# yeyupiaoling/PPASR

Hardware: AMD Instinct MI355X
Metric: audio-seconds/s (RTF^-1) Conformer-streaming fbank, batch32 per GPU, ctc_greedy (higher is better)
Workload: dtype f32; 1 GPU; configs[1]: Conformer streaming (configs/conformer.yml), fbank-80, 32 x 10 s utterances per GPU, V=4233, ctc_greedy, features resident in HBM -> token ids + scores on device; global_batch=32, frames=1000, decoder=ctc_greedy, parallelism=utterance-dp1, pipelined=False, gemm=f32

## Files before the change

### ppasr_amd/csrc/front_fused.hip

```cpp
#include <utility>

#include "conformer_kernels.h"
#include "launch.h"

namespace ppasr {

namespace {
constexpr int kGroupRow[5] = {2, 0, 1, 4, 3};
constexpr int kTapCol[5] = {2, 0, 1, 4, 3};
constexpr int kFactor[5] = {2, 0, 1, 3, 1};
constexpr int quad_slab(int t) { return 4 * kFactor[t / 5] + kFactor[t % 5]; }
constexpr int quad_target(int t) {
  const int g = t / 5, k = t % 5;
  if (g == 0) return k == 0 ? 4 : k <= 2 ? 5 : 4;
  const int a = (g == 1 || g == 2) ? 0 : 2;
  return k == 0 ? (a == 0 ? 5 : 4) : k <= 2 ? a : a + 1;
}
constexpr int quad_fold_src(int t) {
  return t == 1 || t == 5 || t == 21 || t == 23 ? 4 : t == 3 || t == 11 || t == 13 ? 5 : -1;
}
constexpr int quad_fold_mask(int t) {
  return t == 1 ? 0xf : t == 3 ? 0x5 : t == 5 ? 0xa : t == 11 ? 0x2 : t == 13 ? 0x1 : t == 21 ? 0x8 : t == 23 ? 0x4 : 0;
}
constexpr bool quad_fold_clear(int t) { return t == 1 || t == 3 || t == 5 || t == 13 || t == 23; }
static_assert(quad_target(0) == 4 && quad_target(2) == 5 && quad_target(10) == 5 && quad_target(12) == 0 &&
                  quad_target(14) == 1 && quad_target(20) == 4 && quad_target(22) == 2 && quad_target(24) == 3,
              "chunk targets");

template <typename Fn, int... I>
__device__ __forceinline__ void static_for(std::integer_sequence<int, I...>, Fn&& fn) {
  (fn(std::integral_constant<int, I>{}), ...);
}

__host__ __device__ inline int quad_xs_stride(int F, int Q) { return F > 8 * Q + 3 ? F : 8 * Q + 3; }
}

template <bool FROM_Y1>
__device__ __forceinline__ void conv2_quad_body(const float* __restrict__ src, const FrontW& fw, float* __restrict__ out,
                                                int T, int F, int Tp, int F2, int M, int m0, const PadSkip& ps,
                                                const int* __restrict__ tile_tab) {
  constexpr int BP = 32, KC = 128, LD = KC + 4, G = KC / 8, NL = 2, N_CHUNKS = 25;
  constexpr int SLOT = BP * LD;
  const int P = (Tp + 1) >> 1;
  const int Q = (F2 + 1) >> 1;
  int r0 = m0 + blockIdx.x * BP, Mlim = M;
  if (tile_tab) {
    const int t = blockIdx.x, nb = tile_tab[0];
    const int* pre = tile_tab + 1;
    if (t >= pre[nb]) return;
    int lo = 0, hi = nb;
    while (hi - lo > 1) {
      const int mid = (lo + hi) >> 1;
      if (pre[mid] <= t) lo = mid;
      else hi = mid;
    }
    const int S = ps.Tp * ps.unit;
    r0 = lo * S + (t - pre[lo]) * BP;
    Mlim = min(M, (lo + 1) * S);
  } else if (pad_block_skippable(ps, r0, BP, M)) {
    return;
  }
  extern __shared__ __attribute__((aligned(16))) float smem[];
  float* const slot0 = smem;
  float* const slot1 = smem + SLOT;
  f32x4* const y2s = reinterpret_cast<f32x4*>(smem + 2 * SLOT);
  float* const w1s = smem + 2 * SLOT + 5 * NL * 4 * kThreads;
  float* const xs = w1s + 10 * 256;
  const int tid = threadIdx.x, lane = lane_id(), wave = wave_id();
  constexpr int tile_stride = 2 * 16 * G * 64;
  const f32x4* wbase = fw.conv2_wp + (size_t)wave * tile_stride;
  auto seg = [&](int h, int slab) { return wbase + (size_t)(16 * h + slab) * G * 64; };
  BRing<1> ring;
  ring_prime(ring, seg(0, quad_slab(0)), 0);
  const int c4 = tid & 31, rbase = tid >> 5;
  const int bp0 = r0 / Q;
  const int FX = quad_xs_stride(F, Q);
  uint32_t pb = 0;
  int yrow[FROM_Y1 ? NL : 1], yp4[FROM_Y1 ? NL : 1], yq4[FROM_Y1 ? NL : 1];
  if constexpr (!FROM_Y1) {
    for (int idx = tid; idx < 10 * 256; idx += kThreads) w1s[idx] = idx < 9 * 256 ? fw.conv1_w[idx] : fw.conv1_b[idx - 9 * 256];
    const int nbp = (min(r0 + BP, Mlim) - 1) / Q - bp0 + 1;
    for (int idx = tid; idx < nbp * 11 * FX; idx += kThreads) {
      const int fr_row = idx / FX, f = idx - fr_row * FX;
      const int bpl = fr_row / 11, fr = fr_row - 11 * bpl;
      const int bp = bp0 + bpl, b = bp / P, p = bp - b * P;
      const int t = min(8 * p + fr, T - 1);
      xs[idx] = f < F ? (src[((size_t)b * T + t) * F + f] - fw.cmvn_mean[f]) * fw.cmvn_istd[f] : 0.f;
    }
#pragma unroll
    for (int i = 0; i < NL; ++i) {
      const int m = r0 + rbase + 16 * i;
      const int bp = m / Q, q = m - bp * Q;
      const uint32_t v = m < Mlim ? (uint32_t)((bp - bp0) * 11 * FX + 8 * q) : 0xffffu;
      pb |= v << (16 * i);
    }
  } else {
#pragma unroll
    for (int i = 0; i < NL; ++i) {
      const int m = r0 + rbase + 16 * i;
      const int bp = m / Q, q = m - bp * Q, b = bp / P, p = bp - b * P;
      yrow[i] = b * T + 4 * p;
      yp4[i] = 4 * p;
      yq4[i] = m < Mlim ? 4 * q : -1;
    }
  }
  auto pbase = [&](int i) { return (int)((pb >> (16 * i)) & 0xffffu); };
  const int lds_off0 = rbase * LD + 4 * c4;
  float xv[9];
  f32x4 wv[3], bv, ya, yv;
  auto y1_step = [&](int i, int h, int r, int c, int step) {
    const int cc = h * 128 + 4 * c4;
    if constexpr (!FROM_Y1) {
      if (step == 0) {
        const int o = pbase(i);
        const float* p = xs + (o == 0xffff ? 0 : o) + 2 * r * FX + 2 * c;
#pragma unroll
        for (int ii = 0; ii < 3; ++ii)
#pragma unroll
          for (int jj = 0; jj < 3; ++jj) xv[ii * 3 + jj] = p[ii * FX + jj];
        ya = f32x4{0.f, 0.f, 0.f, 0.f};
      } else {
#pragma unroll
        for (int j = 3 * (step - 1); j < 3 * step; ++j)
#pragma unroll
          for (int e = 0; e < 4; ++e) ya[e] = fmaf(wv[j % 3][e], xv[j], ya[e]);
        if (step == 3) {
          ya += bv;
#pragma unroll
          for (int e = 0; e < 4; ++e) ya[e] = pbase(i) != 0xffff ? fmaxf(ya[e], 0.f) : 0.f;
        }
      }
      if (step < 3) {
#pragma unroll
        for (int j = 0; j < 3; ++j) wv[j] = *reinterpret_cast<const f32x4*>(w1s + (3 * step + j) * 256 + cc);
        if (step == 2) bv = *reinterpret_cast<const f32x4*>(w1s + 9 * 256 + cc);
      }
    } else {
      if (step == 0) {
        yv = f32x4{0.f, 0.f, 0.f, 0.f};
        if (yq4[i] >= 0 && yp4[i] + r < T && yq4[i] + c < F)
          yv = *reinterpret_cast<const f32x4*>(src + ((size_t)(yrow[i] + r) * F + yq4[i] + c) * 256 + cc);
      } else if (step == 3) {
        ya = yv;
      }
    }
  };
  auto put = [&](float* buf, int i, const f32x4& v) { *reinterpret_cast<f32x4*>(buf + lds_off0 + i * 16 * LD) = v; };
  auto y2row = [&](int c, int i) -> f32x4& { return y2s[(c * NL + i) * kThreads + tid]; };
  f32x4 z2[NL];
  auto build = [&](auto nc, int g, int h, float* buf) {
    constexpr int n = decltype(nc)::value, grp = n / 5, k = n % 5, r = kGroupRow[grp], c = kTapCol[k];
    const int i = g >> 2, step = g & 3;
    y1_step(i, h, r, c, step);
    if (step != 3) return;
    f32x4 v = ya;
    if constexpr (grp == 0) y2row(c, i) = ya;
    if constexpr (grp == 1 || grp == 3) v = ya - y2row(c, i);
    if constexpr (k == 0) {
      z2[i] = v;
      put(buf, i, v);
    } else if constexpr (k == 1 || k == 3) {
      put(buf, i, v - z2[i]);
    } else {
      put(buf, i, v);
    }
  };
  f32x16 acc[6][1][1];
#pragma unroll
  for (int a = 0; a < 6; ++a) acc_zero(acc[a]);
  auto fold = [&](auto tc, int g) {
    constexpr int t = decltype(tc)::value, fs = quad_fold_src(t), mask = quad_fold_mask(t);
    if constexpr (fs >= 0) {
      const int j = g - 4 * NL;
      int seen = 0;
#pragma unroll
      for (int o = 0; o < 4; ++o) {
        if (!((mask >> o) & 1)) continue;
        if (seen++ == j) {
#pragma unroll
          for (int e = 0; e < 16; ++e) asm volatile("v_add_f32 %0, %0, %1" : "+v"(acc[o][0][0][e]) : "v"(acc[fs][0][0][e]));
        }
      }
      if (quad_fold_clear(t) && j == 4) acc_zero(acc[fs]);
    }
  };
  __syncthreads();
#pragma unroll
  for (int g = 0; g < 4 * NL; ++g) {
    build(std::integral_constant<int, 0>{}, g, 0, slot0);
    __builtin_amdgcn_sched_barrier(0);
  }
  __syncthreads();
  for (int h = 0; h < 2; ++h) {
    asm volatile("" : "+s"(wbase));
    if constexpr (!FROM_Y1) {
      asm volatile("" : "+v"(pb));
    } else {
#pragma unroll
      for (int i = 0; i < NL; ++i) asm volatile("" : "+v"(yrow[i]), "+v"(yp4[i]), "+v"(yq4[i]));
    }
    static_for(std::make_integer_sequence<int, N_CHUNKS>{}, [&](auto tc) {
      constexpr int t = decltype(tc)::value;
      float* const cur = ((t + h) & 1) ? slot1 : slot0;
      float* const nxb = ((t + h) & 1) ? slot0 : slot1;
      const f32x4* nseg = t + 1 < N_CHUNKS ? seg(h, quad_slab(t + 1)) : (h == 0 ? seg(1, quad_slab(0)) : nullptr);
      auto side = [&](int g) {
        if (g < 4 * NL) {
          if constexpr (t + 1 < N_CHUNKS) build(std::integral_constant<int, t + 1>{}, g, h, nxb);
          else if (h == 0) build(std::integral_constant<int, 0>{}, g, 1, nxb);
        } else {
          fold(tc, g);
        }
      };
      rb_gemm<1, 1, G, kPF, decltype(side)>(cur, LD, seg(h, quad_slab(t)), 0, nseg, 0, ring, acc[quad_target(t)], side);
      __syncthreads();
    });
  }
  const int col = wave * 32 + (lane & 31);
  const float b2 = fw.conv2_b[col];
#pragma unroll
  for (int r = 0; r < 16; ++r) {
    const int m = r0 + acc_row(r, lane);
    if (m >= Mlim) continue;
    const int bp = m / Q, q = m - bp * Q, b = bp / P, t0 = 2 * (bp - b * P), f0 = 2 * q;
    float* o = out + ((size_t)(b * Tp + t0) * F2 + f0) * 256 + col;
    const bool f1 = f0 + 1 < F2, t1 = t0 + 1 < Tp;
    o[0] = fmaxf(acc[0][0][0][r] + b2, 0.f);
    if (f1) o[256] = fmaxf(acc[1][0][0][r] + b2, 0.f);
    if (t1) o[(size_t)F2 * 256] = fmaxf(acc[2][0][0][r] + b2, 0.f);
    if (t1 && f1) o[(size_t)F2 * 256 + 256] = fmaxf(acc[3][0][0][r] + b2, 0.f);
  }
}

__global__ __launch_bounds__(kThreads) void k_conv12(const float* __restrict__ feats, FrontW fw, float* __restrict__ out,
                                                     int T, int F, int Tp, int F2, int M, int m0, PadSkip ps,
                                                     const int* __restrict__ tile_tab) {
  conv2_quad_body<false>(feats, fw, out, T, F, Tp, F2, M, m0, ps, tile_tab);
}
__global__ __launch_bounds__(kThreads) void k_conv2_pair(const float* __restrict__ y1, FrontW fw, float* __restrict__ out,
                                                         int T1, int F1, int Tp, int F2, int M, int m0, PadSkip ps,
                                                         const int* __restrict__ tile_tab) {
  conv2_quad_body<true>(y1, fw, out, T1, F1, Tp, F2, M, m0, ps, tile_tab);
}

static int quad_tile_pairs(int Q) { return 31 / Q + 2; }
static size_t quad_lds(bool fused, int F, int F2) {
  const int Q = (F2 + 1) / 2;
  return ((size_t)2 * 32 * 132 + (size_t)5 * 2 * 4 * 512 + (fused ? (size_t)10 * 256 + (size_t)quad_tile_pairs(Q) * 11 * quad_xs_stride(F, Q) : 0)) *
         sizeof(float);
}
bool conv2_quad_supported(const FrontW& fw) { return fw.conv2_wp && fw.conv2_k == 3 && fw.conv2_s == 2; }
bool conv12_supported(const FrontW& fw, int F, int F2) {
  const int Q = (F2 + 1) / 2;
  return conv2_quad_supported(fw) && F2 >= 1 && quad_lds(true, F, F2) <= 160 * 1024 &&
         (size_t)quad_tile_pairs(Q) * 11 * quad_xs_stride(F, Q) < 0xffff;
}

void launch_tile_prefix(const PadSkip& ps, int B, int BM, int* tab, hipStream_t st);

static void launch_quad(bool fused, const float* src, const FrontW& fw, float* y2, int B, int T, int F, int Tp, int F2,
                        hipStream_t st, const PadSkip& ps_frames, int* tile_scratch) {
  const int P = (Tp + 1) / 2, Q = (F2 + 1) / 2;
  PadSkip ps = ps_frames;
  ps.Tp = P;
  ps.mul = 2 * ps_frames.mul;
  ps.slack = (ps_frames.slack + 1) / 2;
  ps.unit = Q;
  const int M = B * P * Q;
  const int* no_tab = nullptr;
#define QUAD(GRID, TAB)                                                                                                  \
  do {                                                                                                                 \
    if (fused)                                                                                                         \
      PPASR_LAUNCH(k_conv12, dim3(GRID), dim3(kThreads), quad_lds(true, F, F2), st, src, fw, y2, T, F, Tp, F2, M, 0, ps, \
                   TAB);                                                                                               \
    else                                                                                                               \
      PPASR_LAUNCH(k_conv2_pair, dim3(GRID), dim3(kThreads), quad_lds(false, F, F2), st, src, fw, y2, T, F, Tp, F2, M, 0, \
                   ps, TAB);                                                                                           \
  } while (0)
  if (ps.lens && tile_scratch) {
    launch_tile_prefix(ps, B, 32, tile_scratch, st);
    QUAD(B * ((P * Q + 31) / 32), (const int*)tile_scratch);
    return;
  }
  QUAD((M + 31) / 32, no_tab);
#undef QUAD
}

void launch_conv12(const float* feats, const FrontW& fw, float* y2, int B, int T, int F, int Tp, int F2, hipStream_t st,
                   const PadSkip& ps_frames, int* tile_scratch) {
  launch_quad(true, feats, fw, y2, B, T, F, Tp, F2, st, ps_frames, tile_scratch);
}
void launch_conv2_quad(const float* y1, const FrontW& fw, float* y2, int B, int T1, int F1, int Tp, int F2, hipStream_t st,
                       const PadSkip& ps_frames, int* tile_scratch) {
  launch_quad(false, y1, fw, y2, B, T1, F1, Tp, F2, st, ps_frames, tile_scratch);
}

hipError_t configure_front_fused_kernels() {
  hipError_t e;
#define SET_LDS(fn)                                                                                              \
  e = hipFuncSetAttribute(reinterpret_cast<const void*>(fn), hipFuncAttributeMaxDynamicSharedMemorySize, 160 * 1024); \
  if (e != hipSuccess) return e;
  SET_LDS(k_conv12);
  SET_LDS(k_conv2_pair);
#undef SET_LDS
  return hipSuccess;
}

}
```

Measured before the change: 58430 audio-s/s.

## Compute fused conv1 im2col tiles with MFMA on four builder waves

The fused conv1+conv2 front-end kernel used to build each conv1 output tile with scalar FMAs on every thread, reading the 3x3 weights from LDS. It now does the 9-tap conv1 (plus bias, via a ones column) as a chain of 32x32x2 f32 MFMAs on the first four waves only. Those waves keep the conv1 weights in registers and load the second half's weights mid-pipeline. The change removes the LDS weight staging and the packed 16-bit row offsets, and it drops the 0xffff limit check. The aim is to cut the VALU cost of rebuilding the conv1 tiles inside the conv2 GEMM loop, at the price of uneven per-wave work, extra register pressure, and a new post/LDS write pattern.

After: 58730 audio-s/s, median of 6. No clear change (+0.5%).

```diff
diff --git a/ppasr_amd/csrc/front_fused.hip b/ppasr_amd/csrc/front_fused.hip
--- a/ppasr_amd/csrc/front_fused.hip
+++ b/ppasr_amd/csrc/front_fused.hip
@@ -64,8 +64,7 @@
   float* const slot0 = smem;
   float* const slot1 = smem + SLOT;
   f32x4* const y2s = reinterpret_cast<f32x4*>(smem + 2 * SLOT);
-  float* const w1s = smem + 2 * SLOT + 5 * NL * 4 * kThreads;
-  float* const xs = w1s + 10 * 256;
+  float* const xs = smem + 2 * SLOT + 5 * NL * 4 * kThreads;
   const int tid = threadIdx.x, lane = lane_id(), wave = wave_id();
   constexpr int tile_stride = 2 * 16 * G * 64;
   const f32x4* wbase = fw.conv2_wp + (size_t)wave * tile_stride;
@@ -75,10 +74,9 @@
   const int c4 = tid & 31, rbase = tid >> 5;
   const int bp0 = r0 / Q;
   const int FX = quad_xs_stride(F, Q);
-  uint32_t pb = 0;
+  int xa[FROM_Y1 ? 1 : 5];
   int yrow[FROM_Y1 ? NL : 1], yp4[FROM_Y1 ? NL : 1], yq4[FROM_Y1 ? NL : 1];
   if constexpr (!FROM_Y1) {
-    for (int idx = tid; idx < 10 * 256; idx += kThreads) w1s[idx] = idx < 9 * 256 ? fw.conv1_w[idx] : fw.conv1_b[idx - 9 * 256];
     const int nbp = (min(r0 + BP, Mlim) - 1) / Q - bp0 + 1;
     for (int idx = tid; idx < nbp * 11 * FX; idx += kThreads) {
       const int fr_row = idx / FX, f = idx - fr_row * FX;
@@ -87,12 +85,13 @@
       const int t = min(8 * p + fr, T - 1);
       xs[idx] = f < F ? (src[((size_t)b * T + t) * F + f] - fw.cmvn_mean[f]) * fw.cmvn_istd[f] : 0.f;
     }
-#pragma unroll
-    for (int i = 0; i < NL; ++i) {
-      const int m = r0 + rbase + 16 * i;
-      const int bp = m / Q, q = m - bp * Q;
-      const uint32_t v = m < Mlim ? (uint32_t)((bp - bp0) * 11 * FX + 8 * q) : 0xffffu;
-      pb |= v << (16 * i);
+    const int m = r0 + (lane & 31);
+    const int bp = m / Q, q = m - bp * Q;
+    const int win = m < Mlim ? (bp - bp0) * 11 * FX + 8 * q : 0;
+#pragma unroll
+    for (int mm = 0; mm < 5; ++mm) {
+      const int k = 2 * mm + (lane >> 5);
+      xa[mm] = win + (k < 9 ? (k / 3) * FX + k % 3 : 0);
     }
   } else {
 #pragma unroll
@@ -104,38 +103,11 @@
       yq4[i] = m < Mlim ? 4 * q : -1;
     }
   }
-  auto pbase = [&](int i) { return (int)((pb >> (16 * i)) & 0xffffu); };
   const int lds_off0 = rbase * LD + 4 * c4;
-  float xv[9];
-  f32x4 wv[3], bv, ya, yv;
+  f32x4 ya, yv;
   auto y1_step = [&](int i, int h, int r, int c, int step) {
     const int cc = h * 128 + 4 * c4;
-    if constexpr (!FROM_Y1) {
-      if (step == 0) {
-        const int o = pbase(i);
-        const float* p = xs + (o == 0xffff ? 0 : o) + 2 * r * FX + 2 * c;
-#pragma unroll
-        for (int ii = 0; ii < 3; ++ii)
-#pragma unroll
-          for (int jj = 0; jj < 3; ++jj) xv[ii * 3 + jj] = p[ii * FX + jj];
-        ya = f32x4{0.f, 0.f, 0.f, 0.f};
-      } else {
-#pragma unroll
-        for (int j = 3 * (step - 1); j < 3 * step; ++j)
-#pragma unroll
-          for (int e = 0; e < 4; ++e) ya[e] = fmaf(wv[j % 3][e], xv[j], ya[e]);
-        if (step == 3) {
-          ya += bv;
-#pragma unroll
-          for (int e = 0; e < 4; ++e) ya[e] = pbase(i) != 0xffff ? fmaxf(ya[e], 0.f) : 0.f;
-        }
-      }
-      if (step < 3) {
-#pragma unroll
-        for (int j = 0; j < 3; ++j) wv[j] = *reinterpret_cast<const f32x4*>(w1s + (3 * step + j) * 256 + cc);
-        if (step == 2) bv = *reinterpret_cast<const f32x4*>(w1s + 9 * 256 + cc);
-      }
-    } else {
+    if constexpr (FROM_Y1) {
       if (step == 0) {
         yv = f32x4{0.f, 0.f, 0.f, 0.f};
         if (yq4[i] >= 0 && yp4[i] + r < T && yq4[i] + c < F)
@@ -148,6 +120,57 @@
   auto put = [&](float* buf, int i, const f32x4& v) { *reinterpret_cast<f32x4*>(buf + lds_off0 + i * 16 * LD) = v; };
   auto y2row = [&](int c, int i) -> f32x4& { return y2s[(c * NL + i) * kThreads + tid]; };
   f32x4 z2[NL];
+  float w1r[FROM_Y1 ? 1 : 5], xin[FROM_Y1 ? 1 : 5];
+  f32x16 c1;
+  f32x4 z4[FROM_Y1 ? 1 : 4];
+  auto load_w1 = [&](int h) {
+    const int ch = h * 128 + 32 * wave + (lane & 31);
+#pragma unroll
+    for (int mm = 0; mm < 5; ++mm) {
+      const int k = 2 * mm + (lane >> 5);
+      w1r[mm] = k < 9 ? fw.conv1_w[k * 256 + ch] : fw.conv1_b[ch];
+    }
+  };
+  const int blane = (lane & 31) * LD + 32 * wave + 4 * (lane >> 5);
+  auto y2quad = [&](int c, int q) -> f32x4& { return y2s[(c * 4 + q) * 256 + tid]; };
+  auto post = [&](auto nc, auto beside, int q, float* buf) {
+    constexpr int n = decltype(nc)::value, grp = n / 5, k = n % 5, c = kTapCol[k];
+    f32x4 v;
+#pragma unroll
+    for (int e = 0; e < 4; ++e) {
+      if constexpr (decltype(beside)::value) asm volatile("v_max_f32 %0, 0, %1" : "=v"(v[e]) : "v"(c1[4 * q + e]));
+      else v[e] = fmaxf(c1[4 * q + e], 0.f);
+    }
+    if constexpr (grp == 0) y2quad(c, q) = v;
+    if constexpr (grp == 1 || grp == 3) v = v - y2quad(c, q);
+    f32x4* const dst = reinterpret_cast<f32x4*>(buf + blane + 8 * q);
+    if constexpr (k == 0) {
+      z4[q] = v;
+      *dst = v;
+    } else if constexpr (k == 1 || k == 3) {
+      *dst = v - z4[q];
+    } else {
+      *dst = v;
+    }
+  };
+  auto build_mfma = [&](auto nc, auto beside, int g, float* buf) {
+    constexpr int n = decltype(nc)::value, r = kGroupRow[n / 5], c = kTapCol[n % 5];
+    if constexpr (!FROM_Y1) {
+      if (g == 0) {
+        const float* p = xs + 2 * r * FX + 2 * c;
+#pragma unroll
+        for (int mm = 0; mm < 5; ++mm) xin[mm] = p[xa[mm]];
+      } else if (g == 1) {
+        c1 = __builtin_amdgcn_mfma_f32_32x32x2f32(w1r[0], xin[0], f32x16{}, 0, 0, 0);
+      } else if (g <= 5) {
+        if (g == 5 && lane >= 32) xin[4] = 1.0f;
+        c1 = __builtin_amdgcn_mfma_f32_32x32x2f32(w1r[g - 1], xin[g - 1], c1, 0, 0, 0);
+      } else if (g <= 7) {
+        post(nc, beside, 2 * (g - 6), buf);
+        post(nc, beside, 2 * (g - 6) + 1, buf);
+      }
+    }
+  };
   auto build = [&](auto nc, int g, int h, float* buf) {
     constexpr int n = decltype(nc)::value, grp = n / 5, k = n % 5, r = kGroupRow[grp], c = kTapCol[k];
     const int i = g >> 2, step = g & 3;
@@ -184,17 +207,21 @@
       if (quad_fold_clear(t) && j == 4) acc_zero(acc[fs]);
     }
   };
+    const bool builder = !FROM_Y1 && wave < 4;
+  if (builder) load_w1(0);
   __syncthreads();
 #pragma unroll
   for (int g = 0; g < 4 * NL; ++g) {
-    build(std::integral_constant<int, 0>{}, g, 0, slot0);
+    if constexpr (FROM_Y1) build(std::integral_constant<int, 0>{}, g, 0, slot0);
+    else if (builder) build_mfma(std::integral_constant<int, 0>{}, std::false_type{}, g, slot0);
     __builtin_amdgcn_sched_barrier(0);
   }
   __syncthreads();
   for (int h = 0; h < 2; ++h) {
     asm volatile("" : "+s"(wbase));
     if constexpr (!FROM_Y1) {
-      asm volatile("" : "+v"(pb));
+#pragma unroll
+      for (int mm = 0; mm < 5; ++mm) asm volatile("" : "+v"(xa[mm]));
     } else {
 #pragma unroll
       for (int i = 0; i < NL; ++i) asm volatile("" : "+v"(yrow[i]), "+v"(yp4[i]), "+v"(yq4[i]));
@@ -206,8 +233,16 @@
       const f32x4* nseg = t + 1 < N_CHUNKS ? seg(h, quad_slab(t + 1)) : (h == 0 ? seg(1, quad_slab(0)) : nullptr);
       auto side = [&](int g) {
         if (g < 4 * NL) {
-          if constexpr (t + 1 < N_CHUNKS) build(std::integral_constant<int, t + 1>{}, g, h, nxb);
-          else if (h == 0) build(std::integral_constant<int, 0>{}, g, 1, nxb);
+          if constexpr (FROM_Y1) {
+            if constexpr (t + 1 < N_CHUNKS) build(std::integral_constant<int, t + 1>{}, g, h, nxb);
+            else if (h == 0) build(std::integral_constant<int, 0>{}, g, 1, nxb);
+          } else if (builder) {
+            if constexpr (t + 1 < N_CHUNKS) build_mfma(std::integral_constant<int, t + 1>{}, std::true_type{}, g, nxb);
+            else if (h == 0) build_mfma(std::integral_constant<int, 0>{}, std::true_type{}, g, nxb);
+            if constexpr (t + 2 == N_CHUNKS) {
+              if (h == 0 && g == 7) load_w1(1);
+            }
+          }
         } else {
           fold(tc, g);
         }
@@ -246,14 +281,12 @@
 static int quad_tile_pairs(int Q) { return 31 / Q + 2; }
 static size_t quad_lds(bool fused, int F, int F2) {
   const int Q = (F2 + 1) / 2;
-  return ((size_t)2 * 32 * 132 + (size_t)5 * 2 * 4 * 512 + (fused ? (size_t)10 * 256 + (size_t)quad_tile_pairs(Q) * 11 * quad_xs_stride(F, Q) : 0)) *
+  return ((size_t)2 * 32 * 132 + (size_t)5 * 2 * 4 * 512 + (fused ? (size_t)quad_tile_pairs(Q) * 11 * quad_xs_stride(F, Q) : 0)) *
          sizeof(float);
 }
 bool conv2_quad_supported(const FrontW& fw) { return fw.conv2_wp && fw.conv2_k == 3 && fw.conv2_s == 2; }
 bool conv12_supported(const FrontW& fw, int F, int F2) {
-  const int Q = (F2 + 1) / 2;
-  return conv2_quad_supported(fw) && F2 >= 1 && quad_lds(true, F, F2) <= 160 * 1024 &&
-         (size_t)quad_tile_pairs(Q) * 11 * quad_xs_stride(F, Q) < 0xffff;
+  return conv2_quad_supported(fw) && F2 >= 1 && quad_lds(true, F, F2) <= 160 * 1024;
 }
 
 void launch_tile_prefix(const PadSkip& ps, int B, int BM, int* tab, hipStream_t st);
```
